# phantomzone-org/poulpy

Measured on NVIDIA B200. Metric: glwe_keyswitch_per_s, higher is better.
Workload: dtype u32 (canonical residues mod four 30-bit primes; i128 big)

## Files before the change

### poulpy_b200/csrc/ntt120_gadget.cu

```cuda
#include <cooperative_groups.h>
#include <stdlib.h>

#include "internal.h"
#include "ntt120.cuh"

namespace cg = cooperative_groups;
using namespace n120;

namespace {

struct GadgetArgs {
    const char *in;  unsigned long long in_bs;
    char *res;       unsigned long long res_bs;
    const uint32_t *ckey;
    const int *key_bits;
    int *ok;
    int in_cols, row_cols, row_col0, R, cols_out;
    int small_size;
    int K, S, res_size;
    int bound_bits;
    int batch;
    int aut_mode, post_size;
    uint32_t aut_pinv;
    uint32_t zero;
    uint32_t m_w[4][4];
    uint32_t nq_w[4];
    unsigned long long half_lo, half_hi;
    uint32_t inv60[4];
    uint32_t crt_ninv[4], crt_ninv_sh[4];
    struct { uint32_t q, c32, c32s, neg64, qni; } prime[4];
};

template <int L> struct GGeo {
    static constexpr int N = 1 << L;
    static constexpr int T = N / 16;
    static constexpr int LV2 = (L >= 12) ? 4 : (L == 11 ? 4 : 3);
    static constexpr int NL2 = (L >= 11) ? 4 : 3;
    static constexpr int NL3 = L - (LV2 + 4) ;
    static constexpr int SG2 = L - LV2 - 4;
    static constexpr bool SIG3 = SG2 == 3;
};

template <int L> __device__ __forceinline__ int swz(int i) {
    int r = i ^ (((i >> 5) & 3) << 2);
    if (GGeo<L>::SIG3) r ^= ((i >> 7) & 3) << 3;
    else r ^= ((i >> 8) & 1) << 4;
    return r;
}

__device__ __forceinline__ void ct_bfz(uint32_t &x, uint32_t &y, uint2 w, uint32_t q, uint32_t z) {
    const uint32_t xr = csub(x, 2 * q);
    const uint32_t t = mul_shoup(y, w.x, w.y, q);
    x = xr + t + z;
    y = xr - t + 2 * q;
}
__device__ __forceinline__ void gs_bfz(uint32_t &x, uint32_t &y, uint2 w, uint32_t q, uint32_t z) {
    const uint32_t s = csub(x + y + z, 2 * q);
    const uint32_t d = x - y + 2 * q;
    x = s;
    y = mul_shoup(d, w.x, w.y, q);
}

template <int NLEV, class TW> __device__ __forceinline__ void ct16(uint32_t (&x)[16], const TW &tw, const uint32_t q, const uint32_t z) {
    if (NLEV >= 4) {
        const uint2 w = tw.get1();
#pragma unroll
        for (int j = 0; j < 8; j++) ct_bfz(x[j], x[j + 8], w, q, z);
    }
    if (NLEV >= 3) {
        uint2 w[2];
        tw.get2(w);
#pragma unroll
        for (int b = 0; b < 2; b++)
// ... 15 lines not shown
        for (int b = 0; b < 8; b++) ct_bfz(x[2 * b], x[2 * b + 1], w[b], q, z);
    }
}
template <int NLEV, class TW> __device__ __forceinline__ void gs16(uint32_t (&x)[16], const TW &tw, const uint32_t q, const uint32_t z) {
    {
        uint2 w[8];
        tw.get8(w);
#pragma unroll
        for (int b = 0; b < 8; b++) gs_bfz(x[2 * b], x[2 * b + 1], w[b], q, z);
    }
    if (NLEV >= 2) {
        uint2 w[4];
        tw.get4(w);
#pragma unroll
        for (int b = 0; b < 4; b++)
#pragma unroll
            for (int j = 0; j < 2; j++) gs_bfz(x[4 * b + j], x[4 * b + j + 2], w[b], q, z);
    }
    if (NLEV >= 3) {
        uint2 w[2];
        tw.get2(w);
#pragma unroll
        for (int b = 0; b < 2; b++)
#pragma unroll
            for (int j = 0; j < 4; j++) gs_bfz(x[8 * b + j], x[8 * b + j + 4], w[b], q, z);
    }
    if (NLEV >= 4) {
        const uint2 w = tw.get1();
#pragma unroll
        for (int j = 0; j < 8; j++) gs_bfz(x[j], x[j + 8], w, q, z);
    }
}

struct TwGlobal {
    const uint2 *tw;
    uint32_t hi;
    __device__ __forceinline__ uint2 get1() const { return __ldg(tw + hi); }
    __device__ __forceinline__ void get2(uint2 (&w)[2]) const {
        const uint4 a = __ldg(reinterpret_cast<const uint4 *>(tw + 2 * hi));
        w[0] = make_uint2(a.x, a.y); w[1] = make_uint2(a.z, a.w);
    }
    __device__ __forceinline__ void get4(uint2 (&w)[4]) const {
        const uint4 *p = reinterpret_cast<const uint4 *>(tw + 4 * hi);
#pragma unroll
        for (int i = 0; i < 2; i++) {
            const uint4 a = __ldg(p + i);
            w[2 * i] = make_uint2(a.x, a.y); w[2 * i + 1] = make_uint2(a.z, a.w);
        }
    }
    __device__ __forceinline__ void get8(uint2 (&w)[8]) const {
        const uint4 *p = reinterpret_cast<const uint4 *>(tw + 8 * hi);
#pragma unroll
        for (int i = 0; i < 4; i++) {
            const uint4 a = __ldg(p + i);
            w[2 * i] = make_uint2(a.x, a.y); w[2 * i + 1] = make_uint2(a.z, a.w);
        }
    }
};
struct TwLast {
    const uint4 *p;
    int T;
    __device__ __forceinline__ uint2 get1() const {
        const uint4 a = __ldg(p);
        return make_uint2(a.x, a.y);
    }
    __device__ __forceinline__ void get2(uint2 (&w)[2]) const {
        const uint4 a = __ldg(p + T);
        w[0] = make_uint2(a.x, a.y); w[1] = make_uint2(a.z, a.w);
    }
    __device__ __forceinline__ void get4(uint2 (&w)[4]) const {
#pragma unroll
        for (int i = 0; i < 2; i++) {
            const uint4 a = __ldg(p + (2 + i) * T);
            w[2 * i] = make_uint2(a.x, a.y); w[2 * i + 1] = make_uint2(a.z, a.w);
        }
    }
    __device__ __forceinline__ void get8(uint2 (&w)[8]) const {
#pragma unroll
        for (int i = 0; i < 4; i++) {
            const uint4 a = __ldg(p + (4 + i) * T);
            w[2 * i] = make_uint2(a.x, a.y); w[2 * i + 1] = make_uint2(a.z, a.w);
        }
    }
};
struct TwRegs {
    uint2 w[16];
    template <class TW> __device__ __forceinline__ void load(const TW &src, const int nlev) {
// ... 65 lines not shown
#pragma unroll
    for (int k = 0; k < NP; k++) tk[k] = ld_cluster(rb[k] + off);
    unsigned long long fr = 1ull << 59;
#pragma unroll
    for (int k = 0; k < NP; k++) fr += (unsigned long long)tk[k] * p.inv60[k];
    const uint32_t e = (uint32_t)(fr >> 60);
    unsigned long long a0 = (unsigned long long)e * p.nq_w[0];
#pragma unroll
    for (int k = 0; k < NP; k++) a0 += (unsigned long long)tk[k] * p.m_w[k][0];
    unsigned long long a1 = (a0 >> 32) + (unsigned long long)e * p.nq_w[1];
#pragma unroll
    for (int k = 0; k < NP; k++) a1 += (unsigned long long)tk[k] * p.m_w[k][1];
    w0 = (uint32_t)a0; w1 = (uint32_t)a1; w2 = 0; w3 = 0;
    if (nwords > 2) {
        unsigned long long a2 = (a1 >> 32) + (unsigned long long)e * p.nq_w[2];
        if (NP == 4) {
#pragma unroll
            for (int k = 0; k < NP; k++) a2 += (unsigned long long)tk[k] * p.m_w[k][2];
        }
        w2 = (uint32_t)a2;
        if (nwords > 3) {
            unsigned long long a3 = (a2 >> 32) + (unsigned long long)e * p.nq_w[3];
            if (NP == 4) {
#pragma unroll
                for (int k = 0; k < NP; k++) a3 += (unsigned long long)tk[k] * p.m_w[k][3];
            }
            w3 = (uint32_t)a3;
        }
    }
}

template <int L, int NP, int NW, bool SMALL>
__device__ __forceinline__ void gadget_tail_narrow(const GadgetArgs &p, const uint32_t (&rb)[NP], const int K, const int t, const int st,
                                                   const int o, const long long *__restrict__ in, long long *__restrict__ res) {
    typedef GGeo<L> Geo;
    constexpr int n = Geo::N, T = Geo::T;
    constexpr int G = NP == 4 ? 4 : 3;
    const int Kb = p.K, S = p.S, cols_out = p.cols_out;
    const int a_start = p.res_size < S ? p.res_size : S;
    const size_t res_ls = (size_t)cols_out * n, in_ls = (size_t)p.in_cols * n;
    const uint32_t kmask32 = (1u << Kb) - 1u, khalf32 = 1u << (Kb - 1);
    const uint32_t hw[4] = {(uint32_t)p.half_lo, (uint32_t)(p.half_lo >> 32), (uint32_t)p.half_hi, (uint32_t)(p.half_hi >> 32)};
#pragma unroll 1
    for (int c0 = K; c0 < 16; c0 += NP * G) {
        bool valid[G];
        uint32_t tk[G][NP];
#pragma unroll
        for (int g = 0; g < G; g++) {
            const int chunk = c0 + g * NP;
            valid[g] = NP == 4 || chunk < 16;
            const uint32_t off = (uint32_t)(o * n + (swz<L>((valid[g] ? chunk : c0) * T) ^ st)) * 4u;
#pragma unroll
            for (int k = 0; k < NP; k++) tk[g][k] = ld_cluster(rb[k] + off);
        }
        const long long *bp = in + (size_t)(S - 1) * in_ls + c0 * T + t;
        long long body[G];
        if (SMALL) {
#pragma unroll
            for (int g = 0; g < G; g++) body[g] = (S - 1 < p.small_size && valid[g]) ? __ldg(bp + g * NP * T) : 0;
        }
        uint32_t w[G][NW];
        {
            unsigned long long a[G];
            uint32_t e[G];
#pragma unroll
            for (int g = 0; g < G; g++) a[g] = 1ull << 59;
#pragma unroll
            for (int k = 0; k < NP; k++) {
                const uint32_t c = p.inv60[k];
#pragma unroll
                for (int g = 0; g < G; g++) a[g] += (unsigned long long)tk[g][k] * c;
            }
#pragma unroll
            for (int g = 0; g < G; g++) e[g] = (uint32_t)(a[g] >> 60);
#pragma unroll
            for (int wi = 0; wi < NW; wi++) {
                const uint32_t nq = p.nq_w[wi], h = hw[wi];
#pragma unroll
                for (int g = 0; g < G; g++) a[g] = (wi ? (a[g] >> 32) : 0ull) + (unsigned long long)e[g] * nq + h;
                if (NP == 4 || wi < 2) {
#pragma unroll
                    for (int k = 0; k < NP; k++) {
                        const uint32_t mw = p.m_w[k][wi];
#pragma unroll
// ... 26 lines not shown
                            : "r"(lo), "r"(hi), "r"(sx));                                                                          \
                }                                                                                                                  \
            }                                                                                                                      \
        }                                                                                                                          \
        if (j_ < a_start) {                                                                                                        \
            _Pragma("unroll") for (int g = 0; g < G; g++)                                                                          \
                if (valid[g]) out_p[g * NP * T] = (long long)((int)(w[g][0] & kmask32) - (int)khalf32);                            \
        }                                                                                                                          \
        out_p -= res_ls;                                                                                                           \
        _Pragma("unroll") for (int g = 0; g < G; g++) {                                                                            \
            _Pragma("unroll") for (int wi = 0; wi + 1 < NW; wi++) w[g][wi] = __funnelshift_r(w[g][wi], w[g][wi + 1], Kb);          \
            w[g][NW - 1] >>= Kb;                                                                                                   \
        }                                                                                                                          \
    }
        long long body2[G];
        int j = S - 1;
#pragma unroll 1
        for (; j >= 1; j -= 2) {
            TAIL_STEP(j, body, body2)
            TAIL_STEP(j - 1, body2, body)
        }
        if (j == 0) TAIL_STEP(0, body, body2)
#undef TAIL_STEP
        long long *zp = res + (size_t)o * n + c0 * T + t;
        for (int j = a_start; j < p.res_size; j++) {
#pragma unroll
            for (int g = 0; g < G; g++)
                if (valid[g]) zp[(size_t)j * res_ls + g * NP * T] = 0;
        }
    }
}

template <int L, int CO>
__device__ __forceinline__ void gadget_mac(uint32_t *__restrict__ sm, const uint4 *__restrict__ ck, const int R, const int (&qa)[4], const uint32_t q,
                                           const uint32_t qni) {
    constexpr int n = GGeo<L>::N, T = GGeo<L>::T;
    constexpr int col_stride = n, row_stride = n * CO;
#pragma unroll 1
    for (int c = 0; c < 4; c++) {
#pragma unroll 1
        for (int r0 = 0; r0 < R; r0 += 4) {
            unsigned long long acc[CO][4];
            const uint4 *ckr = ck + (size_t)r0 * row_stride + c * T;
            const uint32_t *ar = sm + r0 * n + qa[c];
#pragma unroll
            for (int u = 0; u < 4; u++) {
                if (u == 0 || r0 + u < R) {
                    const uint4 a = *reinterpret_cast<const uint4 *>(ar + u * n);
#pragma unroll
                    for (int o = 0; o < CO; o++) {
                        const uint4 m = __ldg(ckr + u * row_stride + o * col_stride);
                        if (u == 0) {
                            acc[o][0] = (unsigned long long)a.x * m.x; acc[o][1] = (unsigned long long)a.y * m.y;
                            acc[o][2] = (unsigned long long)a.z * m.z; acc[o][3] = (unsigned long long)a.w * m.w;
                        } else {
                            acc[o][0] += (unsigned long long)a.x * m.x; acc[o][1] += (unsigned long long)a.y * m.y;
                            acc[o][2] += (unsigned long long)a.z * m.z; acc[o][3] += (unsigned long long)a.w * m.w;
                        }
                    }
                }
            }
#pragma unroll
            for (int o = 0; o < CO; o++) {
                uint4 *dst = reinterpret_cast<uint4 *>(sm + o * n + qa[c]);
                uint32_t y[4];
#pragma unroll
                for (int i = 0; i < 4; i++) y[i] = csub(redc64(acc[o][i], q, qni), 2 * q);
                if (r0 != 0) {
                    const uint4 prev = *dst;
                    y[0] = csub(y[0] + prev.x, 2 * q); y[1] = csub(y[1] + prev.y, 2 * q);
                    y[2] = csub(y[2] + prev.z, 2 * q); y[3] = csub(y[3] + prev.w, 2 * q);
                }
                *dst = make_uint4(y[0], y[1], y[2], y[3]);
            }
        }
    }
}

template <int L, int NP, int NW>
__device__ __forceinline__ void gadget_tail_narrow_aut(const GadgetArgs &p, const uint32_t (&rb)[NP], const int K, const int t, const int o,
                                                       const long long *__restrict__ in, long long *__restrict__ res) {
    typedef GGeo<L> Geo;
    constexpr int n = Geo::N, T = Geo::T;
    constexpr int G = NP == 4 ? 4 : 3;
    const int Kb = p.K, S = p.S, cols_out = p.cols_out, mode = p.aut_mode;
    const int a_start = p.res_size < S ? p.res_size : S;
    const size_t res_ls = (size_t)cols_out * n, in_ls = (size_t)p.in_cols * n;
    const uint32_t kmask32 = (1u << Kb) - 1u, khalf32 = 1u << (Kb - 1);
    const uint32_t hw[4] = {(uint32_t)p.half_lo, (uint32_t)(p.half_lo >> 32), (uint32_t)p.half_hi, (uint32_t)(p.half_hi >> 32)};
    const bool with_small = o == 0 && p.small_size > 0;
#pragma unroll 1
    for (int c0 = K; c0 < 16; c0 += NP * G) {
        bool valid[G], flip[G], negx[G];
        int js[G];
        uint32_t tk[G][NP];
#pragma unroll
        for (int g = 0; g < G; g++) {
            const int chunk = c0 + g * NP;
            valid[g] = NP == 4 || chunk < 16;
            const int jo = (valid[g] ? chunk : c0) * T + t;
            const uint32_t j0 = ((uint32_t)jo * p.aut_pinv) & (uint32_t)(2 * n - 1);
            js[g] = (int)(j0 & (uint32_t)(n - 1));
            flip[g] = j0 >= (uint32_t)n;
            negx[g] = mode == 4 ? false : (mode == 3 ? !flip[g] : flip[g]);
            const uint32_t off = (uint32_t)(o * n + swz<L>(js[g])) * 4u;
#pragma unroll
            for (int k = 0; k < NP; k++) tk[g][k] = ld_cluster(rb[k] + off);
        }
        uint32_t w[G][NW];
        {
            unsigned long long a[G];
            uint32_t e[G];
#pragma unroll
            for (int g = 0; g < G; g++) a[g] = 1ull << 59;
#pragma unroll
            for (int k = 0; k < NP; k++) {
                const uint32_t c = p.inv60[k];
#pragma unroll
                for (int g = 0; g < G; g++) a[g] += (unsigned long long)tk[g][k] * c;
            }
#pragma unroll
            for (int g = 0; g < G; g++) e[g] = (uint32_t)(a[g] >> 60);
#pragma unroll
            for (int wi = 0; wi < NW; wi++) {
                const uint32_t nq = p.nq_w[wi];
#pragma unroll
                for (int g = 0; g < G; g++) a[g] = (wi ? (a[g] >> 32) : 0ull) + (unsigned long long)e[g] * nq;
                if (NP == 4 || wi < 2) {
#pragma unroll
                    for (int k = 0; k < NP; k++) {
                        const uint32_t mw = p.m_w[k][wi];
#pragma unroll
                        for (int g = 0; g < G; g++) a[g] += (unsigned long long)tk[g][k] * mw;
                    }
                }
#pragma unroll
                for (int g = 0; g < G; g++) w[g][wi] = (uint32_t)a[g];
            }
// ... 34 lines not shown
                long long b[G];
#pragma unroll
                for (int g = 0; g < G; g++) b[g] = valid[g] ? __ldg(pp + g * NP * T) : 0;
#pragma unroll
                for (int g = 0; g < G; g++) join(w[g], b[g], mode == 2);
            }
            bp -= in_ls;
            pp -= in_ls;
            if (j < a_start) {
#pragma unroll
                for (int g = 0; g < G; g++) {
                    int d = (int)(w[g][0] & kmask32) - (int)khalf32;
                    if (mode == 4 && flip[g]) d = -d;
                    if (valid[g]) out_p[g * NP * T] = (long long)d;
                }
            }
            out_p -= res_ls;
#pragma unroll
            for (int g = 0; g < G; g++) {
#pragma unroll
                for (int wi = 0; wi + 1 < NW; wi++) w[g][wi] = __funnelshift_r(w[g][wi], w[g][wi + 1], Kb);
                w[g][NW - 1] >>= Kb;
            }
        }
        long long *zp = res + (size_t)o * n + c0 * T + t;
        for (int j = a_start; j < p.res_size; j++) {
#pragma unroll
            for (int g = 0; g < G; g++)
                if (valid[g]) zp[(size_t)j * res_ls + g * NP * T] = 0;
        }
    }
}

template <int L, bool AUT, int NP> __device__ __forceinline__ void gadget_body(const GadgetArgs &p, uint32_t *__restrict__ sm, const uint2 *__restrict__ twf,
                                                             const uint2 *__restrict__ twi, const uint4 *__restrict__ lastf,
                                                             const uint4 *__restrict__ lasti, const int K) {
    typedef GGeo<L> G;
    constexpr int n = G::N, T = G::T;
    const PrimeCtx pc = {p.prime[K].q, p.prime[K].c32, p.prime[K].c32s, p.prime[K].neg64};
    const uint32_t q = pc.q, z = p.zero;
    const int t = threadIdx.x;
    cg::cluster_group cluster = cg::this_cluster();
    const int nclusters = gridDim.x / NP, cid = blockIdx.x / NP;
    const TwGlobal top_f = {twf, 1u}, top_i = {twi, 1u};
    const int R = p.R, cols_out = p.cols_out;
    const int amax_allowed = p.bound_bits - __ldg(p.key_bits);
    const uint32_t sm_base = (uint32_t)__cvta_generic_to_shared(sm);
    uint32_t rb[NP];
#pragma unroll
    for (int k = 0; k < NP; k++) asm volatile("mapa.shared::cluster.u32 %0, %1, %2;" : "=r"(rb[k]) : "r"(sm_base), "r"(k));
    const int st = swz<L>(t);
    const int sb = swz<L>(pass_base<L, G::SG2>(t));
    int qa[4];
#pragma unroll
    for (int c = 0; c < 4; c++) qa[c] = swz<L>(16 * t + 4 * c);
#define P1_ADDR(j) ((st ^ fmask<L>((j) * T)) + (j) * T)
#define P2_ADDR(j) (sb ^ swz<L>((j) << G::SG2))

    for (int ct = cid; ct < p.batch; ct += nclusters) {
        const long long *in = reinterpret_cast<const long long *>(p.in + (size_t)ct * p.in_bs);
        if ((t % NP) == K && (t / NP) < R + p.small_size) {
            const int u = t / NP;
            if (u < p.small_size) {
                prefetch_l2_bulk(in + (size_t)u * p.in_cols * n, n * 8);
            } else if (ct + nclusters < p.batch) {
                const int r = u - p.small_size, limb = r / p.row_cols, col = r % p.row_cols + p.row_col0;
                prefetch_l2_bulk(in + (size_t)nclusters * (p.in_bs / 8) + ((size_t)limb * p.in_cols + col) * n, n * 8);
            }
        }
        uint32_t mag = 0;
        bool too_big = false;
        long long v[16];
        {
            const long long *src = in + (size_t)p.row_col0 * n + t;
#pragma unroll
            for (int j = 0; j < 16; j++) v[j] = __ldg(src + j * T);
        }
        for (int r = 0; r < R; r++) {
            uint32_t x[16];
            uint32_t wide = 0;
#pragma unroll
            for (int j = 0; j < 16; j++) {
                const int lo = (int)v[j], hi = (int)(v[j] >> 32), sg = lo >> 31;
                wide |= (uint32_t)(hi ^ sg);
                mag |= (uint32_t)(lo ^ sg);
                x[j] = (uint32_t)lo + ((uint32_t)sg & (3u * q));
            }
            if (__any_sync(0xffffffffu, wide != 0)) {
                unsigned long long m64 = 0;
#pragma unroll
                for (int j = 0; j < 16; j++) {
                    m64 |= (unsigned long long)(v[j] ^ (v[j] >> 63));
                    x[j] = from_i64_rt(v[j], pc);
                }
                too_big |= amax_allowed < 0 || (m64 >> (amax_allowed > 63 ? 63 : amax_allowed)) != 0;
            }
            if (r + 1 < R) {
                const int limb = (r + 1) / p.row_cols, col = (r + 1) % p.row_cols + p.row_col0;
                const long long *src = in + ((size_t)limb * p.in_cols + col) * n + t;
#pragma unroll
                for (int j = 0; j < 16; j++) v[j] = __ldg(src + j * T);
            }
            ct16<4>(x, top_f, q, z);
            if (r == 0) cl_wait();
            uint32_t *pl = sm + r * n;
#pragma unroll
            for (int j = 0; j < 16; j++) pl[P1_ADDR(j)] = x[j];
        }
        too_big |= amax_allowed < 0 || (amax_allowed < 32 && (mag >> amax_allowed) != 0);
        const int bad = __syncthreads_or(too_big);
        if (bad) {
            if (t == 0 && K == 0) {
                p.ok[ct] = 0;
                p.ok[p.batch + 1 + atomicAdd(p.ok + p.batch, 1)] = ct;
            }
            cl_arrive();
            continue;
        }
        {
            const TwGlobal tw = {twf, (1u << G::LV2) | (uint32_t)(t >> G::SG2)};
            for (int r = 0; r < R; r++) {
                uint32_t *pl = sm + r * n;
                uint32_t x[16];
#pragma unroll
                for (int j = 0; j < 16; j++) x[j] = pl[P2_ADDR(j)];
                ct16<G::NL2>(x, tw, q, z);
#pragma unroll
                for (int j = 0; j < 16; j++) pl[P2_ADDR(j)] = x[j];
            }
        }
        __syncthreads();
        {
            const TwLast tws = {lastf + t, T};
            TwRegs tw;
            tw.load(tws, G::NL3);
            for (int r = 0; r < R; r++) {
                uint32_t *pl = sm + r * n;
                uint32_t x[16];
#pragma unroll
                for (int c = 0; c < 4; c++) {
                    const uint4 v = *reinterpret_cast<const uint4 *>(pl + qa[c]);
                    x[4 * c] = v.x; x[4 * c + 1] = v.y; x[4 * c + 2] = v.z; x[4 * c + 3] = v.w;
                }
                ct16<G::NL3>(x, tw, q, z);
#pragma unroll
                for (int c = 0; c < 4; c++)
                    *reinterpret_cast<uint4 *>(pl + qa[c]) = make_uint4(csub(x[4 * c], 2 * q), csub(x[4 * c + 1], 2 * q),
                                                                        csub(x[4 * c + 2], 2 * q), csub(x[4 * c + 3], 2 * q));
            }
        }
        {
            const uint4 *ck = reinterpret_cast<const uint4 *>(p.ckey) + (size_t)K * (n / 4) + t;
            const uint32_t qni = p.prime[K].qni;
            if (cols_out == 2) gadget_mac<L, 2>(sm, ck, R, qa, q, qni);
            else if (cols_out == 3) gadget_mac<L, 3>(sm, ck, R, qa, q, qni);
            else if (cols_out == 4) gadget_mac<L, 4>(sm, ck, R, qa, q, qni);
            else gadget_mac<L, 1>(sm, ck, R, qa, q, qni);
        }
        {
            const TwLast tws = {lasti + t, T};
            TwRegs tw;
            tw.load(tws, G::NL3);
            for (int o = 0; o < cols_out; o++) {
                uint32_t *pl = sm + o * n;
                uint32_t x[16];
#pragma unroll
                for (int c = 0; c < 4; c++) {
                    const uint4 v = *reinterpret_cast<const uint4 *>(pl + qa[c]);
                    x[4 * c] = v.x; x[4 * c + 1] = v.y; x[4 * c + 2] = v.z; x[4 * c + 3] = v.w;
                }
                gs16<G::NL3>(x, tw, q, z);
#pragma unroll
                for (int c = 0; c < 4; c++) *reinterpret_cast<uint4 *>(pl + qa[c]) = make_uint4(x[4 * c], x[4 * c + 1], x[4 * c + 2], x[4 * c + 3]);
            }
        }
        __syncthreads();
        {
            const TwGlobal tw = {twi, (1u << G::LV2) | (uint32_t)(t >> G::SG2)};
            for (int o = 0; o < cols_out; o++) {
                uint32_t *pl = sm + o * n;
                uint32_t x[16];
#pragma unroll
                for (int j = 0; j < 16; j++) x[j] = pl[P2_ADDR(j)];
                gs16<G::NL2>(x, tw, q, z);
#pragma unroll
                for (int j = 0; j < 16; j++) pl[P2_ADDR(j)] = x[j];
            }
        }
        __syncthreads();
        {
            const uint32_t cn = p.crt_ninv[K], cns = p.crt_ninv_sh[K];
            TwRegs top_r;
            top_r.load(top_i, 4);
            for (int o = 0; o < cols_out; o++) {
                uint32_t *pl = sm + o * n;
                uint32_t x[16];
#pragma unroll
                for (int j = 0; j < 16; j++) x[j] = pl[P1_ADDR(j)];
                gs16<4>(x, top_r, q, z);
#pragma unroll
                for (int j = 0; j < 16; j++) pl[P1_ADDR(j)] = csub(mul_shoup(x[j], cn, cns, q), q);
            }
        }
        cl_arrive();
        cl_wait();
        {
            const int Kb = p.K, S = p.S;
            const int a_start = p.res_size < S ? p.res_size : S;
            const size_t res_ls = (size_t)cols_out * n, in_ls = (size_t)p.in_cols * n;
            const int nwords = (S * Kb + 31) >> 5;
            const bool narrow = Kb < 32;
            const unsigned long long kmask = (1ull << Kb) - 1, khalf = 1ull << (Kb - 1);
            long long *res_ct = reinterpret_cast<long long *>(p.res + (size_t)ct * p.res_bs) + t;
            const long long *in_kt = in + t + (size_t)(S - 1) * in_ls;
            if constexpr (AUT) {
                const int mode = p.aut_mode;
                if (narrow) {
                    long long *res_base = reinterpret_cast<long long *>(p.res + (size_t)ct * p.res_bs);
                    for (int o = 0; o < cols_out; o++) {
                        if (nwords <= 2) gadget_tail_narrow_aut<L, NP, 2>(p, rb, K, t, o, in, res_base);
                        else if (nwords == 3) gadget_tail_narrow_aut<L, NP, 3>(p, rb, K, t, o, in, res_base);
                        else gadget_tail_narrow_aut<L, NP, 4>(p, rb, K, t, o, in, res_base);
                    }
                } else
                for (int o = 0; o < cols_out; o++) {
                    const bool with_small = o == 0 && p.small_size > 0;
#pragma unroll 1
                    for (int chunk = K; chunk < 16; chunk += NP) {
                        const int jo = chunk * T + t;
                        const uint32_t j0 = ((uint32_t)jo * p.aut_pinv) & (uint32_t)(2 * n - 1);
                        const int js = (int)(j0 & (uint32_t)(n - 1));
                        const bool flip = j0 >= (uint32_t)n;
                        const bool negx = mode == 4 ? false : (mode == 3 ? !flip : flip);
                        const uint32_t off = (uint32_t)(o * n + swz<L>(js)) * 4u;
                        uint32_t w0, w1, w2, w3;
                        crt_low_words<NP>(p, rb, off, 4, w0, w1, w2, w3);
                        unsigned long long lo = (unsigned long long)w0 | ((unsigned long long)w1 << 32), hi = (unsigned long long)w2 | ((unsigned long long)w3 << 32);
                        if (negx) {
                            lo = ~lo + 1;
                            hi = ~hi + (lo == 0);
                        }
                        lo += p.half_lo;
                        hi += p.half_hi + (lo < p.half_lo);
                        const long long *bp = in + (size_t)(S - 1) * in_ls + js;
                        const long long *pp = in + (size_t)(S - 1) * in_ls + (size_t)o * n + jo;
                        long long *out_p = reinterpret_cast<long long *>(p.res + (size_t)ct * p.res_bs) + (size_t)(S - 1) * res_ls + (size_t)o * n + jo;
                        for (int j = S - 1; j >= 0; j--) {
                            if (with_small && j < p.small_size) {
                                const long long sv = __ldg(bp);
                                const unsigned long long sl = (unsigned long long)sv, sh = (unsigned long long)(sv >> 63);
                                if (negx) {
                                    const unsigned long long nl = lo - sl;
                                    hi = hi - sh - (lo < sl);
                                    lo = nl;
                                } else {
                                    lo += sl;
                                    hi += sh + (lo < sl);
                                }
                            }
                            if (mode != 4 && j < p.post_size) {
                                const long long sv = __ldg(pp);
                                const unsigned long long sl = (unsigned long long)sv, sh = (unsigned long long)(sv >> 63);
                                if (mode == 2) {
                                    const unsigned long long nl = lo - sl;
                                    hi = hi - sh - (lo < sl);
                                    lo = nl;
                                } else {
                                    lo += sl;
                                    hi += sh + (lo < sl);
                                }
                            }
                            bp -= in_ls;
                            pp -= in_ls;
                            long long d = (long long)(lo & kmask) - (long long)khalf;
                            if (mode == 4 && flip) d = -d;
                            if (j < a_start) *out_p = d;
                            out_p -= res_ls;
                            lo = (lo >> Kb) | (hi << (64 - Kb));
                            hi >>= Kb;
                        }
                        long long *zp = reinterpret_cast<long long *>(p.res + (size_t)ct * p.res_bs) + (size_t)o * n + jo;
                        for (int j = a_start; j < p.res_size; j++) zp[(size_t)j * res_ls] = 0;
                    }
                }
            } else if (narrow) {
                long long *res_base = reinterpret_cast<long long *>(p.res + (size_t)ct * p.res_bs);
                for (int o = 0; o < cols_out; o++) {
                    if (o == 0 && p.small_size > 0) {
                        if (nwords <= 2) gadget_tail_narrow<L, NP, 2, true>(p, rb, K, t, st, o, in, res_base);
                        else if (nwords == 3) gadget_tail_narrow<L, NP, 3, true>(p, rb, K, t, st, o, in, res_base);
                        else gadget_tail_narrow<L, NP, 4, true>(p, rb, K, t, st, o, in, res_base);
                    } else {
                        if (nwords <= 2) gadget_tail_narrow<L, NP, 2, false>(p, rb, K, t, st, o, in, res_base);
                        else if (nwords == 3) gadget_tail_narrow<L, NP, 3, false>(p, rb, K, t, st, o, in, res_base);
                        else gadget_tail_narrow<L, NP, 4, false>(p, rb, K, t, st, o, in, res_base);
                    }
                }
            } else
            for (int o = 0; o < cols_out; o++) {
                const bool with_small = o == 0 && p.small_size > 0;
#pragma unroll 1
                for (int chunk = K; chunk < 16; chunk += NP) {
                    const long long *sp = in_kt + chunk * T;
                    const uint32_t off = (uint32_t)(o * n + (swz<L>(chunk * T) ^ st)) * 4u;
                    uint32_t w0, w1, w2, w3;
                    crt_low_words<NP>(p, rb, off, nwords, w0, w1, w2, w3);
                    unsigned long long lo = ((unsigned long long)w1 << 32) | w0, hi = ((unsigned long long)w3 << 32) | w2;
                    lo += p.half_lo;
                    hi += p.half_hi + (lo < p.half_lo);
                    long long *out_p = res_ct + (size_t)(S - 1) * res_ls + (size_t)o * n + chunk * T;
                    for (int j = S - 1; j >= 0; j--) {
                        if (with_small && j < p.small_size) {
                            const long long sv = __ldg(sp);
                            const unsigned long long sl = (unsigned long long)sv;
                            lo += sl;
                            hi += (unsigned long long)(sv >> 63) + (lo < sl);
                        }
                        sp -= in_ls;
                        if (j < a_start) *out_p = (long long)(lo & kmask) - (long long)khalf;
                        out_p -= res_ls;
                        lo = (lo >> Kb) | (hi << (64 - Kb));
                        hi >>= Kb;
                    }
                    long long *zp = res_ct + (size_t)o * n + chunk * T;
                    for (int j = a_start; j < p.res_size; j++) zp[(size_t)j * res_ls] = 0;
                }
            }
        }
        if (t == 0 && K == 0) p.ok[ct] = 1;
        cl_arrive();
    }
    cl_wait();
#undef P1_ADDR
#undef P2_ADDR
}

template <int L, int MB, bool AUT, int NP>
__global__ void __cluster_dims__(NP, 1, 1) __launch_bounds__(GGeo<L>::T, MB * 256 / GGeo<L>::T)
    ntt120_gadget_kernel(const __grid_constant__ GadgetArgs p, const uint2 *__restrict__ twf, const uint2 *__restrict__ twi,
                         const uint4 *__restrict__ lastf, const uint4 *__restrict__ lasti) {
    extern __shared__ __align__(16) uint32_t smem[];
    constexpr int n = GGeo<L>::N;
    cl_arrive();
    const int k = blockIdx.x % NP;
    gadget_body<L, AUT, NP>(p, smem, twf + (size_t)k * n, twi + (size_t)k * n, lastf + (size_t)k * (n / 2), lasti + (size_t)k * (n / 2), k);
}

struct CollapseArgs2 {
    const char *pmat;
    uint32_t *out;
    int n, R, C, cols_out, S;
    signed char src_row[8], di[8], jmax[8];
    uint32_t c[32][4];
};
__global__ void __launch_bounds__(256) gadget_collapse_key_kernel(CollapseArgs2 p) {
    const int u = blockIdx.x * blockDim.x + threadIdx.x;
    const int n4 = p.n / 4;
    if (u >= n4) return;
    const int k = blockIdx.z;
    const PrimeRt pr(k);
    const int r = blockIdx.y / p.cols_out, col = blockIdx.y % p.cols_out;
    const size_t poly4 = (size_t)4 * n4;
    const int jm = p.jmax[r], di = p.di[r];
    const uint4 *src = reinterpret_cast<const uint4 *>(p.pmat) + ((size_t)p.src_row[r] * p.C + (size_t)di * p.cols_out + col) * poly4 + (size_t)k * n4 + u;
    unsigned long long acc[4] = {0, 0, 0, 0};
    for (int j0 = 0; j0 < jm; j0 += 16) {
        const int j1 = min(j0 + 16, jm);
        for (int j = j0; j < j1; j++) {
            const uint4 v = __ldg(src + (size_t)j * p.cols_out * poly4);
            const unsigned long long cj = p.c[j][k];
            acc[0] += v.x * cj; acc[1] += v.y * cj; acc[2] += v.z * cj; acc[3] += v.w * cj;
        }
#pragma unroll
        for (int i = 0; i < 4; i++) acc[i] = pr.reduce(acc[i]);
    }
    const int T = p.n / 16, t = u >> 2, c = u & 3;
    uint4 *dst = reinterpret_cast<uint4 *>(p.out) + ((size_t)r * p.cols_out + col) * poly4 + (size_t)k * n4 + (size_t)c * T + t;
    *dst = make_uint4((uint32_t)acc[0], (uint32_t)acc[1], (uint32_t)acc[2], (uint32_t)acc[3]);
}

static uint32_t pow2_mod(uint64_t e, uint32_t q) {
    uint64_t r = 1, b = 2;
    while (e) {
        if (e & 1) r = r * b % q;
        b = b * b % q;
        e >>= 1;
    }
    return (uint32_t)r;
}

template <int L, int MB, bool AUT, int NP> int launch_gadget_mb(pgb_module *m, const GadgetArgs &p, size_t smem) {
    typedef GGeo<L> G;
    static bool configured[32] = {};
    cudaLaunchConfig_t cfg = {};
    cfg.blockDim = dim3(G::T);
    cfg.dynamicSmemBytes = smem;
    cfg.stream = m->stream;
    if (!configured[m->device & 31]) {
        PGB_CHECK_CUDA(cudaFuncSetAttribute(ntt120_gadget_kernel<L, MB, AUT, NP>, cudaFuncAttributeMaxDynamicSharedMemorySize, (int)(96 << 10)));
        PGB_CHECK_CUDA(cudaFuncSetAttribute(ntt120_gadget_kernel<L, MB, AUT, NP>, cudaFuncAttributePreferredSharedMemoryCarveout, 100));
        configured[m->device & 31] = true;
    }
    cfg.gridDim = dim3(NP * 148);
    int nc = 0;
    PGB_CHECK_CUDA(cudaOccupancyMaxActiveClusters(&nc, ntt120_gadget_kernel<L, MB, AUT, NP>, &cfg));
    if (nc < 1) {
        pgb_set_error("gadget kernel: no resident cluster fits (smem %zu)", smem);
        return PGB_ERR_UNSUPPORTED;
    }
    const int clusters = p.batch < nc ? p.batch : nc;
    cfg.gridDim = dim3(NP * clusters);
    { ProfScope _ps(m, PROF_GADGET);
    PGB_CHECK_CUDA(cudaLaunchKernelEx(&cfg, ntt120_gadget_kernel<L, MB, AUT, NP>, p, (const uint2 *)m->ntt_fwd, (const uint2 *)m->ntt_inv,
                                      (const uint4 *)m->ntt_last16_f, (const uint4 *)m->ntt_last16_i));
    }
    return PGB_OK;
}
template <int L> int launch_gadget(pgb_module *m, const GadgetArgs &p, size_t smem, int np) {
    if (np == 3) {
        if (p.aut_mode) return launch_gadget_mb<L, 3, true, 3>(m, p, smem);
        return launch_gadget_mb<L, 3, false, 3>(m, p, smem);
    }
    if (p.aut_mode) return launch_gadget_mb<L, 3, true, 4>(m, p, smem);
    if (m->opt[PGB_OPT_GADGET_MB] == 4) return launch_gadget_mb<L, 4, false, 4>(m, p, smem);
    return launch_gadget_mb<L, 3, false, 4>(m, p, smem);
}

}

bool ntt120_gadget_supported(const pgb_module *m, int R, int cols_out, int S, int base2k, int batch) {
    if (m->flavour != PGB_NTT120 || m->log_n < 10 || m->log_n > 12) return false;
    if (opt_on(m, PGB_OPT_NO_GADGET)) return false;
    const int planes = R > cols_out ? R : cols_out;
    if ((size_t)planes * m->n * 4 > (size_t)(96 << 10)) return false;
    if (cols_out < 1 || cols_out > 4 || R < 1 || R > 8) return false;
    if (S < 1 || S > 8 || base2k < 2 || base2k > 62) return false;
    if ((int64_t)S * base2k > 128 || (S - 1) * base2k + 3 >= 118) return false;
    return batch >= 1;
}

int ntt120_gadget_fused(pgb_module *m, const char *in, uint64_t in_bs, int in_cols, int row_cols, int row_col0, int R, const char *pmat,
                        int C, int cols_out, int small_size, char *res, uint64_t res_bs, int res_size, int base2k, int batch, int *ok_out,
                        int dsize, int a_size, int key_rows, int group_limit, int aut_mode, int64_t aut_p, int post_size) {
    const uint64_t n = m->n, poly_bytes = 16 * n;
    const int S = C / cols_out;
    if (dsize < 1) dsize = 1;
    if (dsize == 1) key_rows = R;
    const uint64_t ck_bytes = (uint64_t)R * cols_out * poly_bytes, key_bytes = (uint64_t)key_rows * C * poly_bytes;
    const uint64_t sig[KEY_SIG_WORDS] = {1, (uint64_t)R, (uint64_t)C, (uint64_t)cols_out, (uint64_t)base2k, (uint64_t)dsize, (uint64_t)a_size,
                                         (uint64_t)key_rows, (uint64_t)group_limit, (uint64_t)row_cols};
    const bool pinned = key_is_pinned(m, pmat);
    char *cached = pinned ? (char *)key_cache_find(m, pmat, sig) : nullptr;
    const bool have = cached != nullptr;
    const uint64_t need = have ? 0 : (pinned ? key_bytes : ck_bytes + key_bytes + 256);
    if (m->aux_len < need) {
        if (m->aux_ws) {
            PGB_CHECK_CUDA(cudaStreamSynchronize(m->stream));
            cudaFree(m->aux_ws);
// ... 83 lines not shown
            e >>= 1;
        }
        ninv_n[k] = r;
    }
    for (int k = 0; k < 4; k++) {
        const uint32_t q = qk(k), c32 = (uint32_t)((1ull << 32) % q);
        p.prime[k].q = q;
        p.prime[k].c32 = c32;
        p.prime[k].c32s = (uint32_t)(((unsigned long long)c32 << 32) / q);
        p.prime[k].neg64 = q - (uint32_t)(((unsigned long long)c32 * c32) % q);
        uint32_t qinv = q;
        for (int it = 0; it < 5; it++) qinv *= 2u - q * qinv;
        p.prime[k].qni = 0u - qinv;
        p.nq_w[k] = (uint32_t)(((u128)0 - Q) >> (32 * k));
        if (k >= np) continue;
        const u128 mk = Q / q;
        for (int w = 0; w < 4; w++) p.m_w[k][w] = (uint32_t)(mk >> (32 * w));
        p.inv60[k] = (uint32_t)(((unsigned long long)1 << 60) / q);
        if (np == 4) {
            p.crt_ninv[k] = m->nc.crt_ninv[k];
            p.crt_ninv_sh[k] = m->nc.crt_ninv_sh[k];
        } else {
            uint64_t r = 1, b = (uint64_t)(mk % q), e = q - 2;
            while (e) {
                if (e & 1) r = r * b % q;
                b = b * b % q;
                e >>= 1;
            }
            const uint32_t c = (uint32_t)(r * ninv_n[k] % q);
            p.crt_ninv[k] = c;
            p.crt_ninv_sh[k] = (uint32_t)(((uint64_t)c << 32) / q);
        }
    }
    const int planes = R > cols_out ? R : cols_out;
    const size_t smem = (size_t)planes * n * 4;
    PGB_CHECK_CUDA(cudaMemsetAsync(ok_out + batch, 0, sizeof(int), m->stream));
    switch (m->log_n) {
    case 10: return launch_gadget<10>(m, p, smem, np);
    case 11: return launch_gadget<11>(m, p, smem, np);
    case 12: return launch_gadget<12>(m, p, smem, np);
    default: pgb_set_error("gadget kernel: unsupported n"); return PGB_ERR_UNSUPPORTED;
    }
}
```

Baseline: 3.041 million.

## Stage NTT twiddles in shared memory, ping-pong planes, relax block barriers

Copies the top-level forward and inverse twiddles into static shared memory once per block and reads them from there instead of through the read-only global cache. Plane buffers alternate direction between consecutive batch items (with one spare plane when occupancy allows), so the cluster wait can happen later and the next item's writes avoid the previous item's live planes. Two block-wide barriers between NTT passes are replaced with warp-level syncs, relying on each pass-2 block staying inside one warp. This adds static shared memory per block, which may lower residency, and depends on subtle correctness of the ping-pong addressing and cluster reads.

```diff
diff --git a/poulpy_b200/csrc/ntt120_gadget.cu b/poulpy_b200/csrc/ntt120_gadget.cu
--- a/poulpy_b200/csrc/ntt120_gadget.cu
+++ b/poulpy_b200/csrc/ntt120_gadget.cu
@@ -20,6 +20,7 @@
     int K, S, res_size;
     int bound_bits;
     int batch;
+    int planes;
     int aut_mode, post_size;
     uint32_t aut_pinv;
     uint32_t zero;
@@ -39,6 +40,8 @@
     static constexpr int NL3 = L - (LV2 + 4) ;
     static constexpr int SG2 = L - LV2 - 4;
     static constexpr bool SIG3 = SG2 == 3;
+    static_assert((1 << SG2) <= 32, "a pass-2 block must stay inside one warp");
+    static constexpr int NTW = 1 << (LV2 + 4);
 };
 
 template <int L> __device__ __forceinline__ int swz(int i) {
@@ -120,19 +123,19 @@
     }
 }
 
-struct TwGlobal {
+struct TwShared {
     const uint2 *tw;
     uint32_t hi;
-    __device__ __forceinline__ uint2 get1() const { return __ldg(tw + hi); }
+    __device__ __forceinline__ uint2 get1() const { return tw[hi]; }
     __device__ __forceinline__ void get2(uint2 (&w)[2]) const {
-        const uint4 a = __ldg(reinterpret_cast<const uint4 *>(tw + 2 * hi));
+        const uint4 a = *reinterpret_cast<const uint4 *>(tw + 2 * hi);
         w[0] = make_uint2(a.x, a.y); w[1] = make_uint2(a.z, a.w);
     }
     __device__ __forceinline__ void get4(uint2 (&w)[4]) const {
         const uint4 *p = reinterpret_cast<const uint4 *>(tw + 4 * hi);
 #pragma unroll
         for (int i = 0; i < 2; i++) {
-            const uint4 a = __ldg(p + i);
+            const uint4 a = p[i];
             w[2 * i] = make_uint2(a.x, a.y); w[2 * i + 1] = make_uint2(a.z, a.w);
         }
     }
@@ -140,7 +143,7 @@
         const uint4 *p = reinterpret_cast<const uint4 *>(tw + 8 * hi);
 #pragma unroll
         for (int i = 0; i < 4; i++) {
-            const uint4 a = __ldg(p + i);
+            const uint4 a = p[i];
             w[2 * i] = make_uint2(a.x, a.y); w[2 * i + 1] = make_uint2(a.z, a.w);
         }
     }
@@ -272,7 +275,7 @@
 
 template <int L, int NP, int NW, bool SMALL>
 __device__ __forceinline__ void gadget_tail_narrow(const GadgetArgs &p, const uint32_t (&rb)[NP], const int K, const int t, const int st,
-                                                   const int o, const long long *__restrict__ in, long long *__restrict__ res) {
+                                                   const int o, const int po, const long long *__restrict__ in, long long *__restrict__ res) {
     typedef GGeo<L> Geo;
     constexpr int n = Geo::N, T = Geo::T;
     constexpr int G = NP == 4 ? 4 : 3;
@@ -289,7 +292,7 @@
         for (int g = 0; g < G; g++) {
             const int chunk = c0 + g * NP;
             valid[g] = NP == 4 || chunk < 16;
-            const uint32_t off = (uint32_t)(o * n + (swz<L>((valid[g] ? chunk : c0) * T) ^ st)) * 4u;
+            const uint32_t off = (uint32_t)(po + (swz<L>((valid[g] ? chunk : c0) * T) ^ st)) * 4u;
 #pragma unroll
             for (int k = 0; k < NP; k++) tk[g][k] = ld_cluster(rb[k] + off);
         }
@@ -382,8 +385,8 @@
 }
 
 template <int L, int CO>
-__device__ __forceinline__ void gadget_mac(uint32_t *__restrict__ sm, const uint4 *__restrict__ ck, const int R, const int (&qa)[4], const uint32_t q,
-                                           const uint32_t qni) {
+__device__ __forceinline__ void gadget_mac(uint32_t *__restrict__ pb, const int ps, const uint4 *__restrict__ ck, const int R, const int (&qa)[4],
+                                           const uint32_t q, const uint32_t qni) {
     constexpr int n = GGeo<L>::N, T = GGeo<L>::T;
     constexpr int col_stride = n, row_stride = n * CO;
 #pragma unroll 1
@@ -392,11 +395,11 @@
         for (int r0 = 0; r0 < R; r0 += 4) {
             unsigned long long acc[CO][4];
             const uint4 *ckr = ck + (size_t)r0 * row_stride + c * T;
-            const uint32_t *ar = sm + r0 * n + qa[c];
+            const uint32_t *ar = pb + r0 * ps + qa[c];
 #pragma unroll
             for (int u = 0; u < 4; u++) {
                 if (u == 0 || r0 + u < R) {
-                    const uint4 a = *reinterpret_cast<const uint4 *>(ar + u * n);
+                    const uint4 a = *reinterpret_cast<const uint4 *>(ar + u * ps);
 #pragma unroll
                     for (int o = 0; o < CO; o++) {
                         const uint4 m = __ldg(ckr + u * row_stride + o * col_stride);
@@ -412,7 +415,7 @@
             }
 #pragma unroll
             for (int o = 0; o < CO; o++) {
-                uint4 *dst = reinterpret_cast<uint4 *>(sm + o * n + qa[c]);
+                uint4 *dst = reinterpret_cast<uint4 *>(pb + o * ps + qa[c]);
                 uint32_t y[4];
 #pragma unroll
                 for (int i = 0; i < 4; i++) y[i] = csub(redc64(acc[o][i], q, qni), 2 * q);
@@ -429,7 +432,7 @@
 
 template <int L, int NP, int NW>
 __device__ __forceinline__ void gadget_tail_narrow_aut(const GadgetArgs &p, const uint32_t (&rb)[NP], const int K, const int t, const int o,
-                                                       const long long *__restrict__ in, long long *__restrict__ res) {
+                                                       const int po, const long long *__restrict__ in, long long *__restrict__ res) {
     typedef GGeo<L> Geo;
     constexpr int n = Geo::N, T = Geo::T;
     constexpr int G = NP == 4 ? 4 : 3;
@@ -453,7 +456,7 @@
             js[g] = (int)(j0 & (uint32_t)(n - 1));
             flip[g] = j0 >= (uint32_t)n;
             negx[g] = mode == 4 ? false : (mode == 3 ? !flip[g] : flip[g]);
-            const uint32_t off = (uint32_t)(o * n + swz<L>(js[g])) * 4u;
+            const uint32_t off = (uint32_t)(po + swz<L>(js[g])) * 4u;
 #pragma unroll
             for (int k = 0; k < NP; k++) tk[g][k] = ld_cluster(rb[k] + off);
         }
@@ -554,8 +557,8 @@
     }
 }
 
-template <int L, bool AUT, int NP> __device__ __forceinline__ void gadget_body(const GadgetArgs &p, uint32_t *__restrict__ sm, const uint2 *__restrict__ twf,
-                                                             const uint2 *__restrict__ twi, const uint4 *__restrict__ lastf,
+template <int L, bool AUT, int NP> __device__ __forceinline__ void gadget_body(const GadgetArgs &p, uint32_t *__restrict__ sm, const uint2 *twf,
+                                                             const uint2 *twi, const uint4 *__restrict__ lastf,
                                                              const uint4 *__restrict__ lasti, const int K) {
     typedef GGeo<L> G;
     constexpr int n = G::N, T = G::T;
@@ -564,7 +567,7 @@
     const int t = threadIdx.x;
     cg::cluster_group cluster = cg::this_cluster();
     const int nclusters = gridDim.x / NP, cid = blockIdx.x / NP;
-    const TwGlobal top_f = {twf, 1u}, top_i = {twi, 1u};
+    const TwShared top_f = {twf, 1u}, top_i = {twi, 1u};
     const int R = p.R, cols_out = p.cols_out;
     const int amax_allowed = p.bound_bits - __ldg(p.key_bits);
     const uint32_t sm_base = (uint32_t)__cvta_generic_to_shared(sm);
@@ -579,8 +582,11 @@
 #define P1_ADDR(j) ((st ^ fmask<L>((j) * T)) + (j) * T)
 #define P2_ADDR(j) (sb ^ swz<L>((j) << G::SG2))
 
-    for (int ct = cid; ct < p.batch; ct += nclusters) {
+    for (int ct = cid, it = 0; ct < p.batch; ct += nclusters, it++) {
         const long long *in = reinterpret_cast<const long long *>(p.in + (size_t)ct * p.in_bs);
+        const int pofs = (it & 1) ? (p.planes - 1) * n : 0;
+        const int ps = (it & 1) ? -n : n;
+        uint32_t *const pb = sm + pofs;
         if ((t % NP) == K && (t / NP) < R + p.small_size) {
             const int u = t / NP;
             if (u < p.small_size) {
@@ -624,8 +630,8 @@
                 for (int j = 0; j < 16; j++) v[j] = __ldg(src + j * T);
             }
             ct16<4>(x, top_f, q, z);
-            if (r == 0) cl_wait();
-            uint32_t *pl = sm + r * n;
+            if (r == min(p.planes - cols_out, R - 1)) cl_wait();
+            uint32_t *pl = pb + r * ps;
 #pragma unroll
             for (int j = 0; j < 16; j++) pl[P1_ADDR(j)] = x[j];
         }
@@ -640,9 +646,9 @@
             continue;
         }
         {
-            const TwGlobal tw = {twf, (1u << G::LV2) | (uint32_t)(t >> G::SG2)};
+            const TwShared tw = {twf, (1u << G::LV2) | (uint32_t)(t >> G::SG2)};
             for (int r = 0; r < R; r++) {
-                uint32_t *pl = sm + r * n;
+                uint32_t *pl = pb + r * ps;
                 uint32_t x[16];
 #pragma unroll
                 for (int j = 0; j < 16; j++) x[j] = pl[P2_ADDR(j)];
@@ -651,13 +657,13 @@
                 for (int j = 0; j < 16; j++) pl[P2_ADDR(j)] = x[j];
             }
         }
-        __syncthreads();
+        __syncwarp();
         {
             const TwLast tws = {lastf + t, T};
             TwRegs tw;
             tw.load(tws, G::NL3);
             for (int r = 0; r < R; r++) {
-                uint32_t *pl = sm + r * n;
+                uint32_t *pl = pb + r * ps;
                 uint32_t x[16];
 #pragma unroll
                 for (int c = 0; c < 4; c++) {
@@ -674,17 +680,17 @@
         {
             const uint4 *ck = reinterpret_cast<const uint4 *>(p.ckey) + (size_t)K * (n / 4) + t;
             const uint32_t qni = p.prime[K].qni;
-            if (cols_out == 2) gadget_mac<L, 2>(sm, ck, R, qa, q, qni);
-            else if (cols_out == 3) gadget_mac<L, 3>(sm, ck, R, qa, q, qni);
-            else if (cols_out == 4) gadget_mac<L, 4>(sm, ck, R, qa, q, qni);
-            else gadget_mac<L, 1>(sm, ck, R, qa, q, qni);
+            if (cols_out == 2) gadget_mac<L, 2>(pb, ps, ck, R, qa, q, qni);
+            else if (cols_out == 3) gadget_mac<L, 3>(pb, ps, ck, R, qa, q, qni);
+            else if (cols_out == 4) gadget_mac<L, 4>(pb, ps, ck, R, qa, q, qni);
+            else gadget_mac<L, 1>(pb, ps, ck, R, qa, q, qni);
         }
         {
             const TwLast tws = {lasti + t, T};
             TwRegs tw;
             tw.load(tws, G::NL3);
             for (int o = 0; o < cols_out; o++) {
-                uint32_t *pl = sm + o * n;
+                uint32_t *pl = pb + o * ps;
                 uint32_t x[16];
 #pragma unroll
                 for (int c = 0; c < 4; c++) {
@@ -696,11 +702,11 @@
                 for (int c = 0; c < 4; c++) *reinterpret_cast<uint4 *>(pl + qa[c]) = make_uint4(x[4 * c], x[4 * c + 1], x[4 * c + 2], x[4 * c + 3]);
             }
         }
-        __syncthreads();
+        __syncwarp();
         {
-            const TwGlobal tw = {twi, (1u << G::LV2) | (uint32_t)(t >> G::SG2)};
+            const TwShared tw = {twi, (1u << G::LV2) | (uint32_t)(t >> G::SG2)};
             for (int o = 0; o < cols_out; o++) {
-                uint32_t *pl = sm + o * n;
+                uint32_t *pl = pb + o * ps;
                 uint32_t x[16];
 #pragma unroll
                 for (int j = 0; j < 16; j++) x[j] = pl[P2_ADDR(j)];
@@ -715,7 +721,7 @@
             TwRegs top_r;
             top_r.load(top_i, 4);
             for (int o = 0; o < cols_out; o++) {
-                uint32_t *pl = sm + o * n;
+                uint32_t *pl = pb + o * ps;
                 uint32_t x[16];
 #pragma unroll
                 for (int j = 0; j < 16; j++) x[j] = pl[P1_ADDR(j)];
@@ -740,13 +746,15 @@
                 if (narrow) {
                     long long *res_base = reinterpret_cast<long long *>(p.res + (size_t)ct * p.res_bs);
                     for (int o = 0; o < cols_out; o++) {
-                        if (nwords <= 2) gadget_tail_narrow_aut<L, NP, 2>(p, rb, K, t, o, in, res_base);
-                        else if (nwords == 3) gadget_tail_narrow_aut<L, NP, 3>(p, rb, K, t, o, in, res_base);
-                        else gadget_tail_narrow_aut<L, NP, 4>(p, rb, K, t, o, in, res_base);
+                        const int po = pofs + o * ps;
+                        if (nwords <= 2) gadget_tail_narrow_aut<L, NP, 2>(p, rb, K, t, o, po, in, res_base);
+                        else if (nwords == 3) gadget_tail_narrow_aut<L, NP, 3>(p, rb, K, t, o, po, in, res_base);
+                        else gadget_tail_narrow_aut<L, NP, 4>(p, rb, K, t, o, po, in, res_base);
                     }
                 } else
                 for (int o = 0; o < cols_out; o++) {
                     const bool with_small = o == 0 && p.small_size > 0;
+                    const int po = pofs + o * ps;
 #pragma unroll 1
                     for (int chunk = K; chunk < 16; chunk += NP) {
                         const int jo = chunk * T + t;
@@ -754,7 +762,7 @@
                         const int js = (int)(j0 & (uint32_t)(n - 1));
                         const bool flip = j0 >= (uint32_t)n;
                         const bool negx = mode == 4 ? false : (mode == 3 ? !flip : flip);
-                        const uint32_t off = (uint32_t)(o * n + swz<L>(js)) * 4u;
+                        const uint32_t off = (uint32_t)(po + swz<L>(js)) * 4u;
                         uint32_t w0, w1, w2, w3;
                         crt_low_words<NP>(p, rb, off, 4, w0, w1, w2, w3);
                         unsigned long long lo = (unsigned long long)w0 | ((unsigned long long)w1 << 32), hi = (unsigned long long)w2 | ((unsigned long long)w3 << 32);
@@ -808,23 +816,25 @@
             } else if (narrow) {
                 long long *res_base = reinterpret_cast<long long *>(p.res + (size_t)ct * p.res_bs);
                 for (int o = 0; o < cols_out; o++) {
+                    const int po = pofs + o * ps;
                     if (o == 0 && p.small_size > 0) {
-                        if (nwords <= 2) gadget_tail_narrow<L, NP, 2, true>(p, rb, K, t, st, o, in, res_base);
-                        else if (nwords == 3) gadget_tail_narrow<L, NP, 3, true>(p, rb, K, t, st, o, in, res_base);
-                        else gadget_tail_narrow<L, NP, 4, true>(p, rb, K, t, st, o, in, res_base);
+                        if (nwords <= 2) gadget_tail_narrow<L, NP, 2, true>(p, rb, K, t, st, o, po, in, res_base);
+                        else if (nwords == 3) gadget_tail_narrow<L, NP, 3, true>(p, rb, K, t, st, o, po, in, res_base);
+                        else gadget_tail_narrow<L, NP, 4, true>(p, rb, K, t, st, o, po, in, res_base);
                     } else {
-                        if (nwords <= 2) gadget_tail_narrow<L, NP, 2, false>(p, rb, K, t, st, o, in, res_base);
-                        else if (nwords == 3) gadget_tail_narrow<L, NP, 3, false>(p, rb, K, t, st, o, in, res_base);
-                        else gadget_tail_narrow<L, NP, 4, false>(p, rb, K, t, st, o, in, res_base);
+                        if (nwords <= 2) gadget_tail_narrow<L, NP, 2, false>(p, rb, K, t, st, o, po, in, res_base);
+                        else if (nwords == 3) gadget_tail_narrow<L, NP, 3, false>(p, rb, K, t, st, o, po, in, res_base);
+                        else gadget_tail_narrow<L, NP, 4, false>(p, rb, K, t, st, o, po, in, res_base);
                     }
                 }
             } else
             for (int o = 0; o < cols_out; o++) {
                 const bool with_small = o == 0 && p.small_size > 0;
+                const int po = pofs + o * ps;
 #pragma unroll 1
                 for (int chunk = K; chunk < 16; chunk += NP) {
                     const long long *sp = in_kt + chunk * T;
-                    const uint32_t off = (uint32_t)(o * n + (swz<L>(chunk * T) ^ st)) * 4u;
+                    const uint32_t off = (uint32_t)(po + (swz<L>(chunk * T) ^ st)) * 4u;
                     uint32_t w0, w1, w2, w3;
                     crt_low_words<NP>(p, rb, off, nwords, w0, w1, w2, w3);
                     unsigned long long lo = ((unsigned long long)w1 << 32) | w0, hi = ((unsigned long long)w3 << 32) | w2;
@@ -862,10 +872,17 @@
     ntt120_gadget_kernel(const __grid_constant__ GadgetArgs p, const uint2 *__restrict__ twf, const uint2 *__restrict__ twi,
                          const uint4 *__restrict__ lastf, const uint4 *__restrict__ lasti) {
     extern __shared__ __align__(16) uint32_t smem[];
-    constexpr int n = GGeo<L>::N;
+    typedef GGeo<L> G;
+    constexpr int n = G::N;
+    __shared__ __align__(16) uint2 tw_s[2][G::NTW];
     cl_arrive();
     const int k = blockIdx.x % NP;
-    gadget_body<L, AUT, NP>(p, smem, twf + (size_t)k * n, twi + (size_t)k * n, lastf + (size_t)k * (n / 2), lasti + (size_t)k * (n / 2), k);
+    for (int i = threadIdx.x; i < G::NTW; i += G::T) {
+        tw_s[0][i] = __ldg(twf + (size_t)k * n + i);
+        tw_s[1][i] = __ldg(twi + (size_t)k * n + i);
+    }
+    __syncthreads();
+    gadget_body<L, AUT, NP>(p, smem, tw_s[0], tw_s[1], lastf + (size_t)k * (n / 2), lasti + (size_t)k * (n / 2), k);
 }
 
 struct CollapseArgs2 {
@@ -911,25 +928,45 @@
     return (uint32_t)r;
 }
 
-template <int L, int MB, bool AUT, int NP> int launch_gadget_mb(pgb_module *m, const GadgetArgs &p, size_t smem) {
+template <int L, int MB, bool AUT, int NP> int launch_gadget_mb(pgb_module *m, GadgetArgs p) {
     typedef GGeo<L> G;
+    constexpr int max_planes = (96 << 10) / (4 * G::N);
     static bool configured[32] = {};
+    static int resident[32][max_planes + 1] = {};
     cudaLaunchConfig_t cfg = {};
     cfg.blockDim = dim3(G::T);
-    cfg.dynamicSmemBytes = smem;
     cfg.stream = m->stream;
-    if (!configured[m->device & 31]) {
+    const int dev = m->device & 31;
+    if (!configured[dev]) {
         PGB_CHECK_CUDA(cudaFuncSetAttribute(ntt120_gadget_kernel<L, MB, AUT, NP>, cudaFuncAttributeMaxDynamicSharedMemorySize, (int)(96 << 10)));
         PGB_CHECK_CUDA(cudaFuncSetAttribute(ntt120_gadget_kernel<L, MB, AUT, NP>, cudaFuncAttributePreferredSharedMemoryCarveout, 100));
-        configured[m->device & 31] = true;
+        configured[dev] = true;
     }
     cfg.gridDim = dim3(NP * 148);
-    int nc = 0;
-    PGB_CHECK_CUDA(cudaOccupancyMaxActiveClusters(&nc, ntt120_gadget_kernel<L, MB, AUT, NP>, &cfg));
+    auto clusters_for = [&](int planes, int *nc) -> cudaError_t {
+        if (!resident[dev][planes]) {
+            cfg.dynamicSmemBytes = (size_t)planes * G::N * 4;
+            const cudaError_t e = cudaOccupancyMaxActiveClusters(&resident[dev][planes], ntt120_gadget_kernel<L, MB, AUT, NP>, &cfg);
+            if (e != cudaSuccess) return e;
+            if (!resident[dev][planes]) resident[dev][planes] = -1;
+        }
+        *nc = resident[dev][planes];
+        return cudaSuccess;
+    };
+    const int planes = p.R > p.cols_out ? p.R : p.cols_out;
+    int nc = 0, nc_spare = -1;
+    if (planes > max_planes) {
+        pgb_set_error("gadget kernel: %d planes of %d words exceed the shared memory", planes, G::N);
+        return PGB_ERR_UNSUPPORTED;
+    }
+    PGB_CHECK_CUDA(clusters_for(planes, &nc));
     if (nc < 1) {
-        pgb_set_error("gadget kernel: no resident cluster fits (smem %zu)", smem);
+        pgb_set_error("gadget kernel: no resident cluster fits (%d planes of %d words)", planes, G::N);
         return PGB_ERR_UNSUPPORTED;
     }
+    if (planes < max_planes) PGB_CHECK_CUDA(clusters_for(planes + 1, &nc_spare));
+    p.planes = nc_spare >= nc ? planes + 1 : planes;
+    cfg.dynamicSmemBytes = (size_t)p.planes * G::N * 4;
     const int clusters = p.batch < nc ? p.batch : nc;
     cfg.gridDim = dim3(NP * clusters);
     { ProfScope _ps(m, PROF_GADGET);
@@ -938,14 +975,14 @@
     }
     return PGB_OK;
 }
-template <int L> int launch_gadget(pgb_module *m, const GadgetArgs &p, size_t smem, int np) {
+template <int L> int launch_gadget(pgb_module *m, const GadgetArgs &p, int np) {
     if (np == 3) {
-        if (p.aut_mode) return launch_gadget_mb<L, 3, true, 3>(m, p, smem);
-        return launch_gadget_mb<L, 3, false, 3>(m, p, smem);
-    }
-    if (p.aut_mode) return launch_gadget_mb<L, 3, true, 4>(m, p, smem);
-    if (m->opt[PGB_OPT_GADGET_MB] == 4) return launch_gadget_mb<L, 4, false, 4>(m, p, smem);
-    return launch_gadget_mb<L, 3, false, 4>(m, p, smem);
+        if (p.aut_mode) return launch_gadget_mb<L, 3, true, 3>(m, p);
+        return launch_gadget_mb<L, 3, false, 3>(m, p);
+    }
+    if (p.aut_mode) return launch_gadget_mb<L, 3, true, 4>(m, p);
+    if (m->opt[PGB_OPT_GADGET_MB] == 4) return launch_gadget_mb<L, 4, false, 4>(m, p);
+    return launch_gadget_mb<L, 3, false, 4>(m, p);
 }
 
 }
@@ -1095,13 +1132,11 @@
             p.crt_ninv_sh[k] = (uint32_t)(((uint64_t)c << 32) / q);
         }
     }
-    const int planes = R > cols_out ? R : cols_out;
-    const size_t smem = (size_t)planes * n * 4;
     PGB_CHECK_CUDA(cudaMemsetAsync(ok_out + batch, 0, sizeof(int), m->stream));
     switch (m->log_n) {
-    case 10: return launch_gadget<10>(m, p, smem, np);
-    case 11: return launch_gadget<11>(m, p, smem, np);
-    case 12: return launch_gadget<12>(m, p, smem, np);
+    case 10: return launch_gadget<10>(m, p, np);
+    case 11: return launch_gadget<11>(m, p, np);
+    case 12: return launch_gadget<12>(m, p, np);
     default: pgb_set_error("gadget kernel: unsupported n"); return PGB_ERR_UNSUPPORTED;
     }
 }
```

After: 3.119 million (median of 6 runs). 1.03x the previous value.
